# JackShDr/InfluentialRS

Measured on AMD Instinct MI355X. Metric: scored user-item pairs/sec (whole node), higher is better.
Workload: dtype f32; 1 GPU; c2: n_item=3415, d=128, L=200, H=4, layers=6, ffn=256; one greedy path-search step; users_per_gpu=4096, top_k=100, sweep=bf16 filter + exact f32 re-score, parallelism=single GPU

## Files before the change

influentialrs_amd/csrc/capi.hip:

```cpp
#include <stdlib.h>

#include <new>

#include "irs_internal.h"

int irs_launch_topk_exhaustive(irs_ctx *ctx, const float *xrows, int M, int k, float *val, int64_t *ids0,
                               int32_t *status, hipStream_t s);

static char g_create_err[512] = "";

static inline size_t align_up(size_t v, size_t a) { return (v + a - 1) / a * a; }

extern "C" int irs_abi_version(void) { return IRS_ABI_VERSION; }

extern "C" const char *irs_last_error(const irs_ctx *ctx) { return ctx ? ctx->err : g_create_err; }

extern "C" int irs_create(irs_ctx **out, const irs_dims *dims, const irs_shard *shard) {
    if (!out || !dims) {
        snprintf(g_create_err, sizeof(g_create_err), "irs_create: null argument");
        return IRS_E_INVALID;
    }
    const irs_dims &D = *dims;
#define BAD(...)                                                   \
    do {                                                           \
// ... 10 lines not shown
    if (D.mask_mode != IRS_MASK_IRN && D.mask_mode != IRS_MASK_CAUSAL) BAD("bad mask_mode");
    if (D.mask_mode == IRS_MASK_IRN && (D.u_dim < 1 || D.n_user < 1)) BAD("IRN mask needs user embeddings");
    if (D.max_rows < 1) BAD("max_rows must be >= 1");
    if (D.max_k < 1 || D.max_k > 1024) BAD("max_k must be in [1, 1024]");
    irs_shard sh;
    if (shard) sh = *shard;
    else {
        sh.rank = 0;
        sh.world = 1;
        sh.item_lo = 0;
        sh.item_hi = D.n_item;
    }
    if (sh.item_lo < 0 || sh.item_hi > D.n_item || sh.item_lo >= sh.item_hi) BAD("bad item shard [%lld, %lld)", (long long)sh.item_lo, (long long)sh.item_hi);
    if (sh.item_hi - sh.item_lo > 0x7FFFFFE0LL) BAD("shard too large");
    {
        int dev = 0;
        if (hipGetDevice(&dev) == hipSuccess && (dev < 0 || dev >= IRS_MAX_DEVICES))
            BAD("device ordinal %d: contexts are supported on devices 0 .. %d", dev, IRS_MAX_DEVICES - 1);
    }
#undef BAD
    irs_ctx *c = new (std::nothrow) irs_ctx();
    if (!c) {
        snprintf(g_create_err, sizeof(g_create_err), "out of host memory");
        return IRS_E_INVALID;
    }
    memset(c, 0, sizeof(*c));
    c->dims = D;
    c->shard = sh;
    c->n_local = sh.item_hi - sh.item_lo;
    int dp = 16;
    while (dp < D.d) dp <<= 1;
    c->d_pad = dp;
    c->KS = dp / 16;
    c->n_tiles = (int)((c->n_local + 31) / 32);
    c->max_rows = D.max_rows;
    c->max_seqs = D.max_seqs > 0 ? D.max_seqs : D.max_rows;
    c->m_pad_max = (c->max_rows + 31) & ~31;
    c->lse_slots = 2048;
    {
        const char *e = getenv("IRS_DECODER_GEMM");
        if (e && strcmp(e, "f32") && strcmp(e, "x6") && strcmp(e, "h3")) {
            snprintf(g_create_err, sizeof(g_create_err), "IRS_DECODER_GEMM=%s (expected h3, x6 or f32)", e);
            delete c;
            return IRS_E_INVALID;
        }
        c->use_x6 = e ? (strcmp(e, "f32") == 0 ? IRS_GEMM_F32 : strcmp(e, "x6") == 0 ? IRS_GEMM_X6 : IRS_GEMM_H3) : IRS_GEMM_H3;
        const char *ea = getenv("IRS_ATTN_GEMM");
        if (ea && strcmp(ea, "f32") && strcmp(ea, "h3")) {
            snprintf(g_create_err, sizeof(g_create_err), "IRS_ATTN_GEMM=%s (expected h3 or f32)", ea);
            delete c;
            return IRS_E_INVALID;
        }
        c->use_attn_h3 = ea ? (strcmp(ea, "h3") == 0) : 1;
        const char *es = getenv("IRS_DECODER_SEQ");
        c->use_seq = es ? (strcmp(es, "auto") == 0 ? 2 : (atoi(es) != 0 ? 1 : 0)) : 2;
        const char *ec = getenv("IRS_THR_CARRY");
        c->carry_period = ec ? atoi(ec) : 8;
        if (c->carry_period < 0 || c->carry_period > 1024) c->carry_period = 8;
        const char *eo = getenv("IRS_SHARDED_OVERLAP");
        c->sh_overlap = eo ? (atoi(eo) != 0 ? 1 : 0) : 0;
        const char *er = getenv("IRS_LSE_RING");
        c->lse_no_ring = er ? (strcmp(er, "0") == 0) : 0;
    }
    *out = c;
    return IRS_OK;
}

extern "C" void irs_destroy(irs_ctx *ctx) {
    if (!ctx) return;
    irs_drop_graphs(ctx);
    if (ctx->sh_side) {
        for (int i = 0; i < 8; ++i) (void)hipEventDestroy(ctx->sh_ev[i]);
        (void)hipStreamDestroy(ctx->sh_side);
    }
    if (ctx->prof_ev) {
        for (int i = 0; i < ctx->prof_cap; ++i) {
            hipEventDestroy(ctx->prof_ev[i].a);
            hipEventDestroy(ctx->prof_ev[i].b);
        }
        free(ctx->prof_ev);
    }
    delete ctx;
}

static bool ends_with(const char *s, const char *suf) {
    size_t ls = strlen(s), lf = strlen(suf);
    return ls >= lf && strcmp(s + ls - lf, suf) == 0;
}

extern "C" int irs_bind_weight(irs_ctx *ctx, const char *name, const float *p, int64_t numel) {
    if (!ctx || !name || !p) return IRS_E_INVALID;
    if (strncmp(name, "module.", 7) == 0) name += 7;
    const irs_dims &D = ctx->dims;
    const int64_t d = D.d, F = D.ffn_dim;
    const float **slot = nullptr;
    int64_t want = -1;
    if (!strcmp(name, "item_embedder.weight") || !strcmp(name, "word_embedder.weight")) {
        slot = &ctx->item_emb;
        want = (D.n_item + 1) * d;
    } else if (!strcmp(name, "user_embedder.weight")) {
        slot = &ctx->user_emb;
        want = D.n_user * D.u_dim;
    } else if (!strcmp(name, "pos_embedder.pe")) {
        slot = &ctx->pe;
        want = -2;
        if (numel < (int64_t)D.max_len * d) IRS_FAIL(ctx, IRS_E_INVALID, "pos_embedder.pe too small");
// ... 901 lines not shown
```

influentialrs_amd/csrc/irs_internal.h:

```cpp
#pragma once

#include <hip/hip_runtime.h>
#include <stdint.h>
#include <stdio.h>
#include <string.h>

#include "../../include/irs_hip.h"

#if !defined(IRS_LAB) && (defined(X6_DUMP) || defined(X6_STAMP) || defined(X6_NO_SPLIT) || defined(X6_STAGGER) ||            \
                          defined(X6_NO_MFMA) || defined(X6_NO_READS) || defined(X6_NO_DMA) || defined(X6_NO_BARRIER) ||       \
                          defined(X6_NW) || defined(ATTN_STAMP) || defined(ATTNP_STAMP) ||               \
                          defined(IRS_SMALL_TIMING) || defined(IRS_DIRECT_TIMING) || defined(SWEEP_LAB) || defined(X6D_STAMP) ||              \
                          defined(X6_NO_QKV_STORE) || defined(X6_NSLOT2) || defined(X6_RESID_LATE) || defined(X6_RING4) ||      \
                          defined(X6_SPLIT_ACC4) || defined(SEQ_EXP))
#error "a lab switch (X6_* / ATTN* / IRS_*_TIMING) is defined without IRS_LAB: the product library must be built without them"
#endif

#include <atomic>
#include <functional>
#define IRS_MAX_DEVICES 32
static inline int irs_cur_dev() {
    int d = 0;
    if (hipGetDevice(&d) != hipSuccess || d < 0 || d >= IRS_MAX_DEVICES) d = 0;
    return d;
// ... 12 lines not shown
#define IRS_CAND_BUCKETS 64
#define IRS_CAND_SLOTS 64
#define IRS_CAND_CAP (IRS_CAND_BUCKETS * IRS_CAND_SLOTS)
#define IRS_REFINE_CAP 1024
#define IRS_MAX_GROUPS 2048
#define IRS_MAX_PATH 64
#define IRS_LSE_SLOTS_RING 4096
#define IRS_COOP_FALLBACK_MIN_ITEMS 262144
#define IRS_EXH_SCRATCH_KEYS (64 * 32768)

struct irs_layer_w {
    const float *sa_in_w, *sa_in_b, *sa_out_w, *sa_out_b;
    const float *ca_in_w, *ca_in_b, *ca_out_w, *ca_out_b;
    const float *l1_w, *l1_b, *l2_w, *l2_b;
    const float *n1_w, *n1_b, *n2_w, *n2_b, *n3_w, *n3_b;
};

struct irs_prof_ev {
    hipEvent_t a, b;
};

enum { IRS_STEP_GREEDY = 1, IRS_STEP_BEAM, IRS_STEP_SHARDED_BEAM, IRS_STEP_SHARDED_BEAM_SPLIT };
struct irs_step_key {
    int32_t kind, B, W, P, k, sweep, sample, sample_k;
    uint64_t seed;
    const void *comm, *seq, *user, *hep, *paths, *status;
};
static_assert(sizeof(irs_step_key) == 8 * sizeof(int32_t) + 7 * 8, "irs_step_key is compared with memcmp: no padding");
struct irs_step_graph {
    hipGraphExec_t exec;
    irs_step_key key;
};

struct irs_ctx {
    irs_dims dims;
    irs_shard shard;
    int64_t n_local;
    int d_pad;
    int KS;
    int n_tiles;
    int max_seqs;
    int max_rows;
    int m_pad_max;

    const float *item_emb, *user_emb, *pe, *um_w, *um_b, *proj_w, *proj_b;
    irs_layer_w layer[IRS_MAX_LAYERS];

    uint4 *wp;
    float *bias_pad;
    float *c_l;
    float *wnorm_max;
    float *w_frag16;
    uint4 *w_x6;
    int use_x6;
    bool h3_ok;
    float h3_bound;
    int use_seq;
    bool seq_last;
    int32_t route_last[IRS_ROUTE_FIELDS];
    int route_n;
    int use_attn_h3;
    int lse_no_ring;
    bool finalized;
    bool proj_stale;

    char *ws;
    size_t ws_bytes;
    float *act_x, *act_y, *act_qkv, *act_ao, *act_h, *act_ru;
    float *act_qkv_b1;
    float *act_xf, *act_yf;
    int32_t *tok_row;
    int32_t *seq_cnt, *seq_off, *seq_qrow;
    int32_t *seq_padq;
    int32_t *m_dev;
    int32_t *tile_seq, *tile_idx;
    int32_t *seq_row0, *qrow_tile;
    int32_t *n_wg_dev;
    uint4 *xb;
    float *eps;
    float *thr;
    float *gm;
    unsigned int *cand_cnt;
    unsigned long long *cand;
    float *lse_part;
    int lse_slots;
    float *ref_tmp;
    int thr_valid, thr_M, thr_k, thr_age, carry_period;
    unsigned int *fb_count;
    int32_t *fb_list;
    unsigned long long *exh_keys;
    float *xrows;
    float *top_val;
    int64_t *top_ids;
    int32_t *row_status;
    int32_t *step_ctr;
    int32_t *step_pair;
    int32_t *pos_tmp;
    int64_t *bm_seq[2];
    int32_t *bm_hep[2];
    double *bm_cum[2];
    float *bm_paths[2];
    int64_t *bm_user;
    int64_t *bm_user2;
    int32_t *bm_fin[2];
    int32_t *bm_done[2];
    float *lse_max, *lse_sum;
// ... 318 lines not shown
```

influentialrs_amd/csrc/score.hip:

```cpp
#include <type_traits>

#include "irs_internal.h"

typedef __attribute__((ext_vector_type(16))) float f32x16;
typedef __attribute__((ext_vector_type(8))) __bf16 bf16x8;

#define MODE_PRE 0
#define MODE_EMIT 1
#define MODE_COUNT 2
#define MODE_DENSE 3
#define MODE_LSE 4
#define MODE_CEGRAD 5

struct SweepArgs {
    const uint4 *wp;
    const float *w32;
    const float *bias;
    const uint4 *xb;
    const float *x32;
    int M, M_pad, UT, d;
    int64_t n_local;
    int tile_begin, tile_end, tiles_per_wave, n_strips, n_ublocks;
    int tile_stride;
    int tiles_per_wg;
// ... 1350 lines not shown
}

__global__ void __launch_bounds__(256) k_pack_w(const float *__restrict__ W, const float *__restrict__ b, int64_t n_local,
                                                int n_tiles, int d, int KS, uint4 *__restrict__ wp,
                                                float *__restrict__ bias_pad, unsigned int *__restrict__ wn_bits) {
    int64_t row = (int64_t)blockIdx.x * 4 + (threadIdx.x >> 6);
    int lane = threadIdx.x & 63;
    if (row >= (int64_t)n_tiles * 32) return;
    const int64_t t = row >> 5;
    const int r = (int)(row & 31);
    float ss = 0.f, ssr = 0.f, ssd = 0.f;
    if (lane < 2 * KS) {
        uint4 v = pack8_bf16(W + (size_t)row * d, 8 * lane, d, row < n_local, ss, ssr, ssd);
        wp[((size_t)t * KS + (lane >> 1)) * 64 + (lane & 1) * 32 + r] = v;
    }
    ss = lanes_sum<63>(ss);
    ssr = lanes_sum<63>(ssr);
    ssd = lanes_sum<63>(ssd);
    if (lane == 0) {
        bias_pad[row] = (row < n_local) ? b[row] : -INFINITY;
        if (row < n_local) {
            atomicMax(wn_bits + 0, __float_as_uint(sqrtf(fmaxf(ss, ssr)) * 1.001f));
            atomicMax(wn_bits + 1, __float_as_uint(sqrtf(ssd) * 1.001f));
            atomicMax(wn_bits + 2, __float_as_uint(fabsf(b[row])));
        }
    }
}

#define SEL2_G IRS_MAX_GROUPS
static_assert(SEL2_G == 2048, "k_select_thr_bits: 32 keys per lane");
template <int CTRL>
__device__ __forceinline__ unsigned int dpp_u32(unsigned int v) {
    return (unsigned int)__builtin_amdgcn_update_dpp(0, (int)v, CTRL, 0xF, 0xF, true);
}
__device__ __forceinline__ unsigned int wave_sum_u32(unsigned int v) {
    v += dpp_u32<0xB1>(v);
    v += dpp_u32<0x4E>(v);
    v += dpp_u32<0x141>(v);
    v += dpp_u32<0x140>(v);
    return (unsigned int)__builtin_amdgcn_readlane((int)v, 0) + (unsigned int)__builtin_amdgcn_readlane((int)v, 16) +
           (unsigned int)__builtin_amdgcn_readlane((int)v, 32) + (unsigned int)__builtin_amdgcn_readlane((int)v, 48);
}
__device__ __forceinline__ unsigned int wave_max_u32(unsigned int v) {
    unsigned int o;
    o = dpp_u32<0xB1>(v), v = o > v ? o : v;
    o = dpp_u32<0x4E>(v), v = o > v ? o : v;
    o = dpp_u32<0x141>(v), v = o > v ? o : v;
    o = dpp_u32<0x140>(v), v = o > v ? o : v;
    const unsigned int a = (unsigned int)__builtin_amdgcn_readlane((int)v, 0), b = (unsigned int)__builtin_amdgcn_readlane((int)v, 16);
    const unsigned int c = (unsigned int)__builtin_amdgcn_readlane((int)v, 32), d = (unsigned int)__builtin_amdgcn_readlane((int)v, 48);
    const unsigned int ab = a > b ? a : b, cd = c > d ? c : d;
    return ab > cd ? ab : cd;
}
__global__ void __launch_bounds__(256) k_select_thr_bits(const float *__restrict__ gm, int G, int M, int M_pad, int k,
                                                         const float *__restrict__ eps, float *__restrict__ thr,
                                                         float *__restrict__ traw) {
    constexpr int STRIDE = SEL2_G + 16;
    constexpr int KPL = SEL2_G / 64;
    __shared__ unsigned int sel_lds[4 * STRIDE];
    const int tid = threadIdx.x;
    {
        const int rl = tid & 3, tq = tid >> 2;
        const int row = blockIdx.x * 4 + rl;
        const float *blk = gm + (size_t)blockIdx.x * G * 4 + rl;
        float raw[KPL];
#pragma unroll
        for (int i = 0; i < KPL; ++i) {
            const int g = tq + 64 * i;
            raw[i] = blk[(size_t)(g < G ? g : G - 1) * 4];
        }
#pragma unroll
        for (int i = 0; i < KPL; ++i) asm volatile("" : "+v"(raw[i]));
#pragma unroll
        for (int i = 0; i < KPL; ++i) {
            const int g = tq + 64 * i;
            const unsigned int kk = irs_fkey(raw[i]);
            sel_lds[rl * STRIDE + g] = (g < G && row < M) ? kk : 0u;
        }
    }
    __syncthreads();
    const int lane = tid & 63;
    const int wave = __builtin_amdgcn_readfirstlane(tid >> 6);
    const int row = blockIdx.x * 4 + wave;
    unsigned int key[KPL];
    unsigned int mx = 0u, mnc = 0u;
#pragma unroll
    for (int i = 0; i < KPL; ++i) {
        key[i] = sel_lds[wave * STRIDE + lane + 64 * i];
        mx = key[i] > mx ? key[i] : mx;
        const unsigned int c = (lane + 64 * i < G) ? ~key[i] : 0u;
        mnc = c > mnc ? c : mnc;
    }
    const unsigned int smx = wave_max_u32(mx), smn = ~wave_max_u32(mnc);
    const unsigned int diff = smx ^ smn;
    const int top = diff ? 31 - __builtin_clz(diff) : -1;
    unsigned int prefix = top >= 31 ? 0u : (smx & ~((2u << top) - 1u));
    if (top < 0) prefix = smx;
    for (int bit = top; bit >= 0; --bit) {
        const unsigned int cand = prefix | (1u << bit);
        unsigned int c0 = 0, c1 = 0, c2 = 0, c3 = 0;
#pragma unroll
        for (int i = 0; i < KPL; i += 4) {
            c0 += key[i] >= cand ? 1u : 0u;
            c1 += key[i + 1] >= cand ? 1u : 0u;
            c2 += key[i + 2] >= cand ? 1u : 0u;
            c3 += key[i + 3] >= cand ? 1u : 0u;
        }
        const unsigned int cnt = wave_sum_u32((c0 + c1) + (c2 + c3));
        if (cnt >= (unsigned int)k) prefix = cand;
    }
    if (lane == 0 && row < M_pad) {
// ... 130 lines not shown
            const unsigned long long key = keyfn(j);
            if (key > s_thr) {
                const unsigned int slot = atomicAdd(&s_n, 1u);
                buf[slot] = key;
            }
        }
        __syncthreads();
        if (s_n > EXH_BUF - 256) {
            const unsigned int n = s_n;
            for (int i = n + tid; i < EXH_BUF; i += 256) buf[i] = 0ull;
            bitonic_desc(buf, EXH_BUF);
            if (tid == 0) {
                s_n = (n < (unsigned int)k) ? n : k;
                if (n >= (unsigned int)k) s_thr = buf[k - 1];
            }
            __syncthreads();
        }
    }
    const unsigned int n = s_n;
    for (int i = n + tid; i < EXH_BUF; i += 256) buf[i] = 0ull;
    bitonic_desc(buf, EXH_BUF);
    __syncthreads();
    return n < (unsigned int)k ? n : (unsigned int)k;
}

__global__ void __launch_bounds__(256) k_exh_strips(const float *__restrict__ x, int d, const float *__restrict__ W,
                                                    const float *__restrict__ bias, int64_t n_local, int k, int n_strips,
                                                    const unsigned int *__restrict__ fb_count, const int32_t *__restrict__ fb_list,
                                                    unsigned long long *__restrict__ exh_keys) {
    __shared__ unsigned long long buf[EXH_BUF];
    __shared__ float xs[256];
    unsigned int nfb = *fb_count;
    if (nfb == 0u) return;
    if (nfb > EXH_FB_MAX) nfb = EXH_FB_MAX;
    const int strip = blockIdx.x;
    const int64_t per = (n_local + n_strips - 1) / n_strips;
    const int64_t j0 = (int64_t)strip * per, j1 = (j0 + per < n_local) ? j0 + per : n_local;
    for (unsigned int fi = blockIdx.y; fi < nfb; fi += gridDim.y) {
        const int row = fb_list[fi];
        __syncthreads();
        for (int i = threadIdx.x; i < d; i += 256) xs[i] = x[(size_t)row * d + i];
        __syncthreads();
        const unsigned int n = exh_select(
            [&](int64_t j) -> unsigned long long {
                const float e = irs_chain(xs, W + (size_t)j * d, bias[j], d);
                return ((unsigned long long)irs_fkey(e) << 32) | (0xFFFFFFFFu - (unsigned int)j);
            },
            j0, j1, k, buf);
        unsigned long long *o = exh_keys + ((size_t)fi * n_strips + strip) * k;
        for (int i = threadIdx.x; i < k; i += 256) o[i] = i < (int)n ? buf[i] : 0ull;
    }
}

__global__ void __launch_bounds__(256) k_refine(const float *__restrict__ x, int d, const float *__restrict__ W,
                                                const float *__restrict__ bias, const unsigned int *__restrict__ cnt,
                                                const unsigned long long *__restrict__ cand,
                                                const float *__restrict__ eps, const float *__restrict__ traw, int k,
                                                int64_t item_lo, int64_t n_local, float *__restrict__ val,
                                                int64_t *__restrict__ ids, int32_t *__restrict__ status,
                                                unsigned int *__restrict__ fb_count, int32_t *__restrict__ fb_list) {
    __shared__ __attribute__((aligned(16))) unsigned long long ckeys[IRS_CAND_CAP + 2];
    unsigned long long *rkeys = ckeys;
    __shared__ unsigned int hist[256];
    __shared__ float xs[256];
    __shared__ unsigned int boff[IRS_CAND_BUCKETS + 1];
    __shared__ unsigned int s_prefix, s_k, s_nr, s_above, s_over;
    const int row = blockIdx.x, tid = threadIdx.x;
    constexpr int PER = IRS_CAND_BUCKETS * IRS_CAND_SLOTS / 256;
    unsigned long long cv[PER];
#pragma unroll
    for (int j = 0; j < PER; ++j) {
        const int idx = tid + 256 * j;
        cv[j] = cand[((size_t)row * IRS_CAND_BUCKETS + idx / IRS_CAND_SLOTS) * IRS_CAND_SLOTS + idx % IRS_CAND_SLOTS];
    }
    for (int i = tid; i < d; i += 256) xs[i] = x[(size_t)row * d + i];
    if (tid < IRS_CAND_BUCKETS) hist[tid] = cnt[(size_t)row * IRS_CAND_BUCKETS + tid];
    __syncthreads();
    if (tid < 64) {
        const unsigned int cb = hist[tid] & ~IRS_CAND_OVERFLOW;
        const unsigned int cl = cb > IRS_CAND_SLOTS ? IRS_CAND_SLOTS : cb;
        unsigned int incl = cl;
#pragma unroll
        for (int o = 1; o < 64; o <<= 1) {
            const unsigned int t = __shfl_up(incl, o, 64);
            if (tid >= o) incl += t;
        }
        boff[tid] = incl - cl;
        if (tid == 63) boff[IRS_CAND_BUCKETS] = incl;
        const unsigned long long ov = __ballot((hist[tid] & IRS_CAND_OVERFLOW) != 0u);
        if (tid == 0) {
            s_over = ov ? 1u : 0u;
            s_prefix = 0;
            s_k = k;
            s_nr = 0;
            s_above = 0;
        }
    }
    __syncthreads();
    if (s_over) {
        if (tid == 0) status[row] |= IRS_ROW_FALLBACK;
        if (fb_count) {
            if (tid == 0) fb_list[atomicAdd(fb_count, 1u)] = row;
            return;
        }
        exhaustive_row(x, d, W, bias, n_local, item_lo, k, row, val, ids, status, ckeys, xs, true);
        return;
    }
    const unsigned int c = boff[IRS_CAND_BUCKETS];
#pragma unroll
    for (int j = 0; j < PER; ++j) {
        const int idx = tid + 256 * j;
        const int b = idx / IRS_CAND_SLOTS, sl = idx % IRS_CAND_SLOTS;
        if ((unsigned int)sl < boff[b + 1] - boff[b]) ckeys[boff[b] + sl] = cv[j];
    }
    __syncthreads();
    const float t1 = traw[row];
    if (t1 > -INFINITY) {
        unsigned int mine = 0;
        for (int i = tid; i < (int)c; i += 256) mine += (irs_unkey((unsigned int)(ckeys[i] >> 32)) >= t1) ? 1u : 0u;
        if (mine) atomicAdd(&s_above, mine);
// ... 31 lines not shown
            }
            __syncthreads();
            if (tid < 64) radix_find_bin(hist, s_k, tid, shift, &s_prefix, &s_k);
            __syncthreads();
        }
        thr2 = irs_unkey(s_prefix) - 2.0f * eps[row];
    }
    {
        constexpr int PERC = IRS_CAND_CAP / 256;
        unsigned int keep[PERC];
#pragma unroll
        for (int j = 0; j < PERC; ++j) {
            const int i = tid + 256 * j;
            keep[j] = 0xFFFFFFFFu;
            if (i < (int)c) {
                const unsigned long long key = ckeys[i];
                if (irs_unkey((unsigned int)(key >> 32)) >= thr2) keep[j] = (unsigned int)key;
            }
        }
        __syncthreads();
#pragma unroll
        for (int j = 0; j < PERC; ++j)
            if (keep[j] != 0xFFFFFFFFu) rkeys[atomicAdd(&s_nr, 1u)] = (unsigned long long)keep[j];
    }
    __syncthreads();
    const unsigned int nr = s_nr;
    for (int i = tid; i < (int)nr; i += 256) {
        unsigned int j = (unsigned int)rkeys[i];
        float e = irs_chain(xs, W + (size_t)j * d, bias[j], d);
        rkeys[i] = ((unsigned long long)irs_fkey(e) << 32) | (0xFFFFFFFFu - j);
    }
    if ((nr & 1) && tid == 0) rkeys[nr] = 0ull;
    __syncthreads();
    {
        const ulonglong2 *r2 = reinterpret_cast<const ulonglong2 *>(rkeys);
        for (int i = tid; i < (int)nr; i += 256) {
            const unsigned long long me = rkeys[i];
            int above = 0;
            for (int j = 0; j < (int)(nr + 1) / 2; ++j) {
                const ulonglong2 v = r2[j];
                above += (v.x > me) + (v.y > me);
            }
            if (above < k) {
                val[(size_t)row * k + above] = irs_unkey((unsigned int)(me >> 32));
                ids[(size_t)row * k + above] = item_lo + (int64_t)(0xFFFFFFFFu - (unsigned int)me);
            }
        }
        for (int i = (int)nr + tid; i < k; i += 256) {
            val[(size_t)row * k + i] = -INFINITY;
            ids[(size_t)row * k + i] = -1;
        }
    }
    if (tid == 0 && (int)nr < k) status[row] |= IRS_ROW_FEWER_THAN_K;
}

#define DIRECT_MAX_ITEMS 4096
#define DIRECT_TILE 64
#define DIRECT_MAX_D 256
#ifdef IRS_DIRECT_TIMING
__device__ unsigned long long g_direct_t[16];
#define DSTAMP(i) do { if (threadIdx.x == 0) tstamp[i] = __builtin_amdgcn_s_memtime(); } while (0)
#else
#define DSTAMP(i)
#endif
#define DIRECT_ROWS 8
template <int MODE>
__global__ void __launch_bounds__(256) k_topk_direct(const float *__restrict__ x, int d, const float *__restrict__ W,
                                                     const float *__restrict__ bias, int n_local, int64_t item_lo, int k,
                                                     unsigned long long *__restrict__ gkeys, unsigned int *__restrict__ arrive,
                                                     float *__restrict__ val, int64_t *__restrict__ ids,
                                                     int32_t *__restrict__ status, irs_path_args pa, int M) {
    __shared__ __attribute__((aligned(16))) float tile[DIRECT_TILE * (DIRECT_MAX_D + 4)];
    __shared__ __attribute__((aligned(16))) unsigned long long rkeys[IRS_REFINE_CAP + 2];
    __shared__ __attribute__((aligned(16))) float xs[(MODE == 1 ? DIRECT_ROWS : 1) * DIRECT_MAX_D];
    __shared__ __attribute__((aligned(16))) unsigned long long tmax[256];
    __shared__ unsigned int wsum[4];
    __shared__ unsigned int s_last, s_thr;
    const int row = MODE == 1 ? blockIdx.y * DIRECT_ROWS : blockIdx.y, tid = threadIdx.x, lane = tid & 63, wave = tid >> 6;
#ifdef IRS_DIRECT_TIMING
    unsigned long long tstamp[10];
#endif
    DSTAMP(0);
    unsigned int *gk = reinterpret_cast<unsigned int *>(gkeys + (size_t)row * IRS_CAND_CAP);
    if constexpr (MODE != 2) {
    const bool vec = (d & 3) == 0;
    const int S = vec ? ((d & 7) ? d : d + 4) : (d | 1);
    const int j0 = blockIdx.x * DIRECT_TILE;
    const int nj = min(DIRECT_TILE, n_local - j0);
    const int d4 = d >> 2;
    if (vec) {
        for (int i = tid; i < nj * d4; i += 256) {
            const int jj = i / d4, c4 = i - jj * d4;
            *reinterpret_cast<float4 *>(tile + jj * S + 4 * c4) = reinterpret_cast<const float4 *>(W + (size_t)j0 * d)[i];
        }
    } else {
        for (int i = tid; i < nj * d; i += 256) {
            const int jj = i / d, c = i - jj * d;
            tile[jj * S + c] = W[(size_t)j0 * d + i];
        }
    }
    if constexpr (MODE == 1) {
        for (int i = tid; i < DIRECT_ROWS * d; i += 256) {
            const int rr = i / d, c = i - rr * d;
            xs[rr * DIRECT_MAX_D + c] = (row + rr < M) ? x[(size_t)(row + rr) * d + c] : 0.f;
        }
        __syncthreads();
// ... 494 lines not shown
    }
    const bool xreg = a.UT == 1 && KS == 16;
    const int UB = xreg ? 1 : ub_f32(KS);
    a.n_ublocks = (a.UT + UB - 1) / UB;
    dim3 grid(((a.n_strips + 7) / 8) * 8 * a.n_ublocks);
    const size_t lds = (size_t)UB * KS * 2048 + EMIT_Q_BYTES;
#define L_(KS_, UB_, XR_)                                                                                                 \
    do {                                                                                                                  \
        IRS_ONCE_PER_DEVICE((void)hipFuncSetAttribute(reinterpret_cast<const void *>(k_lse_f32<KS_, UB_, EMIT, XR_>),     \
                                                      hipFuncAttributeMaxDynamicSharedMemorySize, (int)lds));             \
        hipLaunchKernelGGL((k_lse_f32<KS_, UB_, EMIT, XR_>), grid, dim3(256), lds, s, a);                                 \
    } while (0)
    switch (KS) {
    case 2: L_(2, 8, false); break;
    case 4: L_(4, 8, false); break;
    case 8: L_(8, 4, false); break;
    case 16: if (xreg) L_(16, 1, true); else L_(16, 2, false); break;
    default: IRS_FAIL(ctx, IRS_E_UNSUPPORTED, "unsupported d_pad %d", ctx->d_pad);
    }
#undef L_
    IRS_CHECK_HIP(ctx, hipGetLastError());
    return IRS_OK;
}

int irs_launch_pack_w(irs_ctx *ctx, hipStream_t s) {
    IRS_CHECK_HIP(ctx, hipMemsetAsync(ctx->wnorm_max, 0, 4 * sizeof(float), s));
    int64_t rows = (int64_t)ctx->n_tiles * 32;
    hipLaunchKernelGGL(k_pack_w, dim3((unsigned)((rows + 3) / 4)), dim3(256), 0, s, ctx->proj_w, ctx->proj_b,
                       ctx->n_local, ctx->n_tiles, ctx->dims.d, ctx->KS, ctx->wp,
                       ctx->bias_pad, reinterpret_cast<unsigned int *>(ctx->wnorm_max));
    IRS_CHECK_HIP(ctx, hipGetLastError());
    return IRS_OK;
}

bool irs_topk_is_direct(const irs_ctx *ctx, int M, int k) {
    return M <= 1024 && ctx->n_local <= DIRECT_MAX_ITEMS && k <= 256 && ctx->dims.d <= DIRECT_MAX_D;
}

enum TopkForm {
    TOPK_DIRECT1,
    TOPK_DIRECT2,
    TOPK_SWEPT,
};
struct TopkPlan {
    TopkForm form;
    bool fused_lse;
    bool lse_after;
    bool reuse_thr;
    bool coop_fb;
    int stride;
    int nt0;
    int tpw0;
    int r_sel;
};

static TopkPlan topk_plan(const irs_ctx *ctx, const float *xrows, int M, int k, int sweep, bool want_lse, int carry) {
    TopkPlan p{};
    if (irs_topk_is_direct(ctx, M, k)) {
        p.form = M <= 32 ? TOPK_DIRECT1 : TOPK_DIRECT2;
        p.lse_after = want_lse;
        return p;
    }
    p.form = TOPK_SWEPT;
    SweepArgs a;
    sweep_common(ctx, a, xrows, M);
    p.fused_lse = want_lse && sweep == IRS_SWEEP_BF16 && lse_fast_ok(ctx, a);
    p.lse_after = want_lse && !p.fused_lse;
    p.coop_fb = ctx->n_local >= IRS_COOP_FALLBACK_MIN_ITEMS && ctx->exh_keys != nullptr;
    const int nt = ctx->n_tiles;
    p.reuse_thr = carry && ctx->carry_period > 0 && sweep == IRS_SWEEP_BF16 && !p.fused_lse && ctx->thr_valid && ctx->thr_M == M &&
                  ctx->thr_k == k && ctx->thr_age + 1 < ctx->carry_period && nt >= 2 * 8 * 1024;
    if (p.reuse_thr) return p;
    int nt0 = nt >= 16 * 1024 ? nt / 16 : nt / 8;
    if (nt0 < 1024) nt0 = 1024;
    if (nt0 > nt) nt0 = nt;
    p.stride = nt / nt0;
    p.nt0 = (nt + p.stride - 1) / p.stride;
    p.tpw0 = (p.nt0 + 1023) / 1024;
    p.r_sel = k;
    if (p.stride > 1) {
        p.r_sel = ((p.stride >= 16 ? 4 : 3) * k + p.stride - 1) / p.stride;
        if (p.r_sel < 8) p.r_sel = 8;
        if (p.r_sel > k) p.r_sel = k;
    }
    return p;
}

static int topk_direct(irs_ctx *ctx, const TopkPlan &p, const float *xrows, int M, int k, float *val, int64_t *ids0,
                       int32_t *status, const irs_path_args *path, hipStream_t s) {
    irs_prof_begin(ctx, IRS_PROF_REFINE, s);
    const unsigned int tiles = (unsigned)((ctx->n_local + DIRECT_TILE - 1) / DIRECT_TILE);
    unsigned int *arrive = reinterpret_cast<unsigned int *>(ctx->step_ctr) + 8;
    const irs_path_args pa = path ? *path : irs_path_args{};
    if (p.form == TOPK_DIRECT1)
        hipLaunchKernelGGL(k_topk_direct<0>, dim3(tiles, M), dim3(256), 0, s, xrows, ctx->dims.d, ctx->proj_w, ctx->proj_b,
                           (int)ctx->n_local, ctx->shard.item_lo, k, ctx->cand, arrive, val, ids0, status, pa, M);
    else {
        hipLaunchKernelGGL(k_topk_direct<1>, dim3(tiles, (M + DIRECT_ROWS - 1) / DIRECT_ROWS), dim3(256), 0, s, xrows, ctx->dims.d,
                           ctx->proj_w, ctx->proj_b, (int)ctx->n_local, ctx->shard.item_lo, k, ctx->cand, arrive, val, ids0,
                           status, irs_path_args{}, M);
        hipLaunchKernelGGL(k_topk_direct<2>, dim3(1, M), dim3(256), 0, s, xrows, ctx->dims.d, ctx->proj_w, ctx->proj_b,
                           (int)ctx->n_local, ctx->shard.item_lo, k, ctx->cand, arrive, val, ids0, status, pa, M);
    }
    irs_prof_end(ctx, IRS_PROF_REFINE, s, 2.0 * ctx->dims.d * (double)M * (double)ctx->n_local, 0.0);
    IRS_CHECK_HIP(ctx, hipGetLastError());
    return IRS_OK;
}

static int topk_prep(irs_ctx *ctx, const TopkPlan &p, const float *xrows, int M, int M_pad, int sweep, int32_t *status,
                     hipStream_t s) {
    static_assert(IRS_CAND_BUCKETS == 64, "k_prep_x resets one bucket counter per lane");
    if (sweep == IRS_SWEEP_BF16) {
        const float acc_factor = (float)(ctx->d_pad + 8) * 2.384185791015625e-07f;
        hipLaunchKernelGGL(k_prep_x, dim3((M_pad + 3) / 4), dim3(256), 0, s, xrows, M, M_pad, ctx->dims.d, ctx->KS,
                           ctx->xb, ctx->eps, ctx->wnorm_max, acc_factor, ctx->cand_cnt, status, p.coop_fb ? ctx->fb_count : nullptr,
                           p.reuse_thr ? ctx->thr : nullptr, p.reuse_thr ? ctx->ref_tmp : nullptr);
    } else {
        IRS_CHECK_HIP(ctx, hipMemsetAsync(status, 0, sizeof(int32_t) * M, s));
        IRS_CHECK_HIP(ctx, hipMemsetAsync(ctx->cand_cnt, 0, sizeof(unsigned int) * (size_t)M_pad * IRS_CAND_BUCKETS, s));
        hipLaunchKernelGGL(k_zero_eps, dim3((M_pad + 255) / 256), dim3(256), 0, s, ctx->eps, M_pad);
    }
    IRS_CHECK_HIP(ctx, hipGetLastError());
    return IRS_OK;
}

static int topk_select(irs_ctx *ctx, const TopkPlan &p, SweepArgs &a, int M, int sweep, hipStream_t s) {
    sweep_decompose(a, 0, ctx->n_tiles, 1, p.tpw0, p.stride);
    const int G = 2 * a.n_strips * 4;
    if (G > SEL2_G) IRS_FAIL(ctx, IRS_E_UNSUPPORTED, "pre-pass groups %d > %d", G, SEL2_G);
    a.gm = ctx->gm;
    a.n_groups = G;
    irs_prof_begin(ctx, IRS_PROF_SWEEP, s);
    const int rc = sweep == IRS_SWEEP_BF16 ? launch_sweep_bf16<MODE_PRE>(ctx, a, s) : launch_sweep_f32<MODE_PRE>(ctx, a, s);
    irs_prof_end(ctx, IRS_PROF_SWEEP, s, 2.0 * ctx->dims.d * (double)M * p.nt0 * 32.0,
                 (double)p.nt0 * 32.0 * ctx->d_pad * (sweep == IRS_SWEEP_BF16 ? 2.0 : 4.0));
    if (rc) return rc;
    hipLaunchKernelGGL(k_select_thr_bits, dim3((a.M_pad + 3) / 4), dim3(256), 0, s, ctx->gm, G, M, a.M_pad, p.r_sel, ctx->eps,
                       ctx->thr, ctx->ref_tmp);
    IRS_CHECK_HIP(ctx, hipGetLastError());
    return IRS_OK;
}

static int topk_emit(irs_ctx *ctx, const TopkPlan &p, SweepArgs &a, int M, int sweep, float *lse_max, float *lse_sum,
                     hipStream_t s) {
    a.thr = ctx->thr;
    a.cnt = ctx->cand_cnt;
    a.cand = ctx->cand;
    int lse_slots = 0, rc;
    if (p.fused_lse) {
        if ((rc = lse_decompose(ctx, a, &lse_slots))) return rc;
    } else {
        const int UB = sweep == IRS_SWEEP_BF16 ? ub_bf16(ctx->KS) : ub_f32(ctx->KS);
        sweep_decompose(a, 0, ctx->n_tiles, (a.UT + UB - 1) / UB, 0);
    }
    const double flops = 2.0 * ctx->dims.d * (double)M * (double)ctx->n_local;
    const double bytes = (double)ctx->n_tiles * 32.0 * ctx->d_pad * ((sweep == IRS_SWEEP_BF16 && !p.fused_lse) ? 2.0 : 4.0);
    irs_prof_begin(ctx, IRS_PROF_SWEEP, s);
    irs_prof_begin(ctx, IRS_PROF_SWEEP_EMIT, s);
    if (p.fused_lse) rc = launch_lse_f32<true>(ctx, a, s);
    else if (sweep == IRS_SWEEP_BF16) rc = launch_sweep_bf16<MODE_EMIT>(ctx, a, s);
    else rc = launch_sweep_f32<MODE_EMIT>(ctx, a, s);
    irs_prof_end(ctx, IRS_PROF_SWEEP, s, flops, bytes);
    irs_prof_end(ctx, IRS_PROF_SWEEP_EMIT, s, flops, bytes);
    if (rc) return rc;
    if (p.fused_lse) {
        hipLaunchKernelGGL(k_lse_reduce, dim3(M), dim3(256), 0, s, ctx->lse_part, lse_slots, a.M_pad, M, lse_max, lse_sum);
        IRS_CHECK_HIP(ctx, hipGetLastError());
    }
    return IRS_OK;
}

static int topk_refine(irs_ctx *ctx, const TopkPlan &p, const float *xrows, int M, int k, int sweep, float *val, int64_t *ids0,
                       int32_t *status, hipStream_t s) {
    const int d = ctx->dims.d;
    irs_prof_begin(ctx, IRS_PROF_REFINE, s);
    if (p.coop_fb && sweep != IRS_SWEEP_BF16) IRS_CHECK_HIP(ctx, hipMemsetAsync(ctx->fb_count, 0, sizeof(unsigned int), s));
    hipLaunchKernelGGL(k_refine, dim3(M), dim3(256), 0, s, xrows, d, ctx->proj_w, ctx->proj_b, ctx->cand_cnt, ctx->cand,
                       ctx->eps, ctx->ref_tmp, k, ctx->shard.item_lo, ctx->n_local, val, ids0, status,
                       p.coop_fb ? ctx->fb_count : nullptr, ctx->fb_list);
    if (p.coop_fb) {
        int ns = EXH_STRIPS;
        while (ns > 1 && (long long)ns * k > EXH_KEYS_PER_ROW) ns >>= 1;
        hipLaunchKernelGGL(k_exh_strips, dim3(ns, 4), dim3(256), 0, s, xrows, d, ctx->proj_w, ctx->proj_b, ctx->n_local, k, ns,
                           ctx->fb_count, ctx->fb_list, ctx->exh_keys);
        hipLaunchKernelGGL(k_exh_merge, dim3(EXH_FB_MAX), dim3(256), 0, s, xrows, d, ctx->proj_w, ctx->proj_b, ctx->n_local,
                           ctx->shard.item_lo, k, ns, ctx->fb_count, ctx->fb_list, ctx->exh_keys, val, ids0, status);
    }
    irs_prof_end(ctx, IRS_PROF_REFINE, s, 0.0, 0.0);
    IRS_CHECK_HIP(ctx, hipGetLastError());
    return IRS_OK;
}

int irs_launch_topk(irs_ctx *ctx, const float *xrows, int M, int k, int sweep, float *val, int64_t *ids0,
                    int32_t *status, hipStream_t s, const irs_path_args *path, float *lse_max, float *lse_sum, int carry) {
    const TopkPlan p = topk_plan(ctx, xrows, M, k, sweep, lse_max != nullptr, carry);
    if (path && p.form == TOPK_SWEPT) IRS_FAIL(ctx, IRS_E_STATE, "fused path step needs the direct top-k");
    int rc;
    if (p.form != TOPK_SWEPT) {
        if ((rc = topk_direct(ctx, p, xrows, M, k, val, ids0, status, path, s))) return rc;
    } else {
        SweepArgs a;
        sweep_common(ctx, a, xrows, M);
        if ((rc = topk_prep(ctx, p, xrows, M, a.M_pad, sweep, status, s))) return rc;
        if (p.reuse_thr) ++ctx->thr_age;
        else {
            if ((rc = topk_select(ctx, p, a, M, sweep, s))) return rc;
            ctx->thr_valid = sweep == IRS_SWEEP_BF16, ctx->thr_M = M, ctx->thr_k = k, ctx->thr_age = 0;
        }
        if ((rc = topk_emit(ctx, p, a, M, sweep, lse_max, lse_sum, s))) return rc;
        if ((rc = topk_refine(ctx, p, xrows, M, k, sweep, val, ids0, status, s))) return rc;
    }
    return p.lse_after ? irs_launch_lse(ctx, xrows, M, lse_max, lse_sum, s) : IRS_OK;
}

int irs_launch_topk_exhaustive(irs_ctx *ctx, const float *xrows, int M, int k, float *val, int64_t *ids0,
                               int32_t *status, hipStream_t s) {
    IRS_CHECK_HIP(ctx, hipMemsetAsync(status, 0, sizeof(int32_t) * M, s));
    hipLaunchKernelGGL(k_exhaustive, dim3(M), dim3(256), 0, s, xrows, ctx->dims.d, ctx->proj_w, ctx->proj_b,
                       ctx->n_local, ctx->shard.item_lo, k, 0, val, ids0, status);
    IRS_CHECK_HIP(ctx, hipGetLastError());
    return IRS_OK;
}

int irs_launch_gather(irs_ctx *ctx, const float *xrows, int M, const int64_t *ids0, int g, float *out, hipStream_t s) {
    hipLaunchKernelGGL(k_gather, dim3(M), dim3(64), 0, s, xrows, ctx->dims.d, ctx->proj_w, ctx->proj_b,
                       ctx->shard.item_lo, ctx->n_local, ids0, g, out);
    IRS_CHECK_HIP(ctx, hipGetLastError());
    return IRS_OK;
}

int irs_launch_count_before(irs_ctx *ctx, const float *xrows, int M, const float *ref_score, const int64_t *ref_id0,
                            const int64_t *excl, int n_excl, int64_t *count, hipStream_t s) {
// ... 137 lines not shown
```

Measured before the change: 2.208 billion pairs/s.

## Add wave-per-row top-k refine and narrow threshold select for small group counts

Adds k_refine_wave, which handles four rows per block with one wavefront each. Each wave gathers the candidates, finds the threshold by radix bit search using wave reductions, re-scores the survivors in f32, and ranks them by counting. Rows that overflow or hit the capacity limit fall back to the existing block-per-row refine. A templated k_select_thr_bits with a smaller keys-per-lane count is used when the group count fits. Both paths are on by default for the bf16 stride-1 non-LSE sweep and can be turned off with IRS_TOPK_ONE_SWEEP=0. The aim is to cut per-row block overhead and __syncthreads in refine; the cost is a smaller per-wave candidate capacity and an O(nr²) rank step.

```diff
diff --git a/influentialrs_amd/csrc/capi.hip b/influentialrs_amd/csrc/capi.hip
--- a/influentialrs_amd/csrc/capi.hip
+++ b/influentialrs_amd/csrc/capi.hip
@@ -86,6 +86,13 @@
             return IRS_E_INVALID;
         }
         c->use_attn_h3 = ea ? (strcmp(ea, "h3") == 0) : 1;
+        const char *et = getenv("IRS_TOPK_ONE_SWEEP");
+        if (et && strcmp(et, "0") && strcmp(et, "1")) {
+            snprintf(g_create_err, sizeof(g_create_err), "IRS_TOPK_ONE_SWEEP=%s (expected 0 or 1)", et);
+            delete c;
+            return IRS_E_INVALID;
+        }
+        c->topk_tight = et ? (strcmp(et, "1") == 0) : 1;
         const char *es = getenv("IRS_DECODER_SEQ");
         c->use_seq = es ? (strcmp(es, "auto") == 0 ? 2 : (atoi(es) != 0 ? 1 : 0)) : 2;
         const char *ec = getenv("IRS_THR_CARRY");
diff --git a/influentialrs_amd/csrc/irs_internal.h b/influentialrs_amd/csrc/irs_internal.h
--- a/influentialrs_amd/csrc/irs_internal.h
+++ b/influentialrs_amd/csrc/irs_internal.h
@@ -88,6 +88,7 @@
     float *wnorm_max;
     float *w_frag16;
     uint4 *w_x6;
+    int topk_tight;
     int use_x6;
     bool h3_ok;
     float h3_bound;
diff --git a/influentialrs_amd/csrc/score.hip b/influentialrs_amd/csrc/score.hip
--- a/influentialrs_amd/csrc/score.hip
+++ b/influentialrs_amd/csrc/score.hip
@@ -1426,11 +1426,12 @@
     const unsigned int ab = a > b ? a : b, cd = c > d ? c : d;
     return ab > cd ? ab : cd;
 }
+template <int KPL>
 __global__ void __launch_bounds__(256) k_select_thr_bits(const float *__restrict__ gm, int G, int M, int M_pad, int k,
                                                          const float *__restrict__ eps, float *__restrict__ thr,
                                                          float *__restrict__ traw) {
-    constexpr int STRIDE = SEL2_G + 16;
-    constexpr int KPL = SEL2_G / 64;
+    static_assert(KPL % 4 == 0 && KPL * 64 <= SEL2_G, "four partial counts; at most IRS_MAX_GROUPS keys");
+    constexpr int STRIDE = KPL * 64 + 16;
     __shared__ unsigned int sel_lds[4 * STRIDE];
     const int tid = threadIdx.x;
     {
@@ -1667,20 +1668,18 @@
     }
 }
 
-__global__ void __launch_bounds__(256) k_refine(const float *__restrict__ x, int d, const float *__restrict__ W,
-                                                const float *__restrict__ bias, const unsigned int *__restrict__ cnt,
-                                                const unsigned long long *__restrict__ cand,
-                                                const float *__restrict__ eps, const float *__restrict__ traw, int k,
-                                                int64_t item_lo, int64_t n_local, float *__restrict__ val,
-                                                int64_t *__restrict__ ids, int32_t *__restrict__ status,
-                                                unsigned int *__restrict__ fb_count, int32_t *__restrict__ fb_list) {
-    __shared__ __attribute__((aligned(16))) unsigned long long ckeys[IRS_CAND_CAP + 2];
+__device__ __forceinline__ void refine_row(const float *__restrict__ x, int d, const float *__restrict__ W,
+                                           const float *__restrict__ bias, const unsigned int *__restrict__ cnt,
+                                           const unsigned long long *__restrict__ cand, const float *__restrict__ eps,
+                                           const float *__restrict__ traw, int k, int64_t item_lo, int64_t n_local,
+                                           float *__restrict__ val, int64_t *__restrict__ ids, int32_t *__restrict__ status,
+                                           unsigned int *__restrict__ fb_count, int32_t *__restrict__ fb_list, const int row,
+                                           unsigned long long *ckeys, float *xs) {
     unsigned long long *rkeys = ckeys;
     __shared__ unsigned int hist[256];
-    __shared__ float xs[256];
     __shared__ unsigned int boff[IRS_CAND_BUCKETS + 1];
     __shared__ unsigned int s_prefix, s_k, s_nr, s_above, s_over;
-    const int row = blockIdx.x, tid = threadIdx.x;
+    const int tid = threadIdx.x;
     constexpr int PER = IRS_CAND_BUCKETS * IRS_CAND_SLOTS / 256;
     unsigned long long cv[PER];
 #pragma unroll
@@ -1818,6 +1817,149 @@
         }
     }
     if (tid == 0 && (int)nr < k) status[row] |= IRS_ROW_FEWER_THAN_K;
+}
+
+__global__ void __launch_bounds__(256) k_refine(const float *__restrict__ x, int d, const float *__restrict__ W,
+                                                const float *__restrict__ bias, const unsigned int *__restrict__ cnt,
+                                                const unsigned long long *__restrict__ cand,
+                                                const float *__restrict__ eps, const float *__restrict__ traw, int k,
+                                                int64_t item_lo, int64_t n_local, float *__restrict__ val,
+                                                int64_t *__restrict__ ids, int32_t *__restrict__ status,
+                                                unsigned int *__restrict__ fb_count, int32_t *__restrict__ fb_list) {
+    __shared__ __attribute__((aligned(16))) unsigned long long ckeys[IRS_CAND_CAP + 2];
+    __shared__ float xs[256];
+    refine_row(x, d, W, bias, cnt, cand, eps, traw, k, item_lo, n_local, val, ids, status, fb_count, fb_list, (int)blockIdx.x,
+               ckeys, xs);
+}
+
+#define RW_CAP (IRS_CAND_CAP / 4)
+#define RW_PER (RW_CAP / 64)
+__device__ __forceinline__ void wave_lds_sync() {
+    __builtin_amdgcn_fence(__ATOMIC_ACQ_REL, "wavefront");
+    __builtin_amdgcn_wave_barrier();
+}
+__global__ void __launch_bounds__(256) k_refine_wave(const float *__restrict__ x, int d, const float *__restrict__ W,
+                                                     const float *__restrict__ bias, const unsigned int *__restrict__ cnt,
+                                                     const unsigned long long *__restrict__ cand,
+                                                     const float *__restrict__ eps, const float *__restrict__ traw, int k,
+                                                     int64_t item_lo, int64_t n_local, float *__restrict__ val,
+                                                     int64_t *__restrict__ ids, int32_t *__restrict__ status,
+                                                     unsigned int *__restrict__ fb_count, int32_t *__restrict__ fb_list, int M) {
+    __shared__ __attribute__((aligned(16))) unsigned long long ckeys[IRS_CAND_CAP + 2];
+    __shared__ float xs4[4 * 256];
+    __shared__ unsigned int woff[4][IRS_CAND_BUCKETS + 1];
+    __shared__ unsigned int s_slow[4];
+    const int tid = threadIdx.x, lane = tid & 63;
+    const int wave = __builtin_amdgcn_readfirstlane(tid >> 6);
+    const int row = blockIdx.x * 4 + wave;
+    unsigned long long *wk = ckeys + wave * RW_CAP;
+    float *xs = xs4 + wave * 256;
+    bool slow = false;
+    if (row < M) {
+        const unsigned int h = cnt[(size_t)row * IRS_CAND_BUCKETS + lane];
+        for (int i = lane; i < d; i += 64) xs[i] = x[(size_t)row * d + i];
+        const float t1 = traw[row], e2 = eps[row];
+        const unsigned int cb = h & ~IRS_CAND_OVERFLOW;
+        const unsigned int cl = cb > IRS_CAND_SLOTS ? IRS_CAND_SLOTS : cb;
+        unsigned int incl = cl;
+#pragma unroll
+        for (int o = 1; o < 64; o <<= 1) {
+            const unsigned int t = __shfl_up(incl, o, 64);
+            if (lane >= o) incl += t;
+        }
+        woff[wave][lane] = incl - cl;
+        if (lane == 63) woff[wave][IRS_CAND_BUCKETS] = incl;
+        const unsigned int c = (unsigned int)__builtin_amdgcn_readlane((int)incl, 63);
+        slow = __ballot((h & IRS_CAND_OVERFLOW) != 0u) != 0ull || c >= RW_CAP;
+        if (!slow) {
+            wave_lds_sync();
+            unsigned int khi[RW_PER], klo[RW_PER];
+#pragma unroll
+            for (int j = 0; j < RW_PER; ++j) {
+                const unsigned int i = (unsigned int)lane + 64u * j;
+                khi[j] = 0u;
+                klo[j] = 0u;
+                if (64u * j < c && i < c) {
+                    unsigned int b = 0u;
+#pragma unroll
+                    for (unsigned int st = IRS_CAND_BUCKETS / 2; st; st >>= 1)
+                        if (woff[wave][b + st] <= i) b += st;
+                    const unsigned long long key = cand[((size_t)row * IRS_CAND_BUCKETS + b) * IRS_CAND_SLOTS + (i - woff[wave][b])];
+                    khi[j] = (unsigned int)(key >> 32);
+                    klo[j] = (unsigned int)key;
+                }
+            }
+            if (t1 > -INFINITY) {
+                unsigned int mine = 0u;
+#pragma unroll
+                for (int j = 0; j < RW_PER; ++j)
+                    if (64u * j < c) mine += ((unsigned int)lane + 64u * j < c && irs_unkey(khi[j]) >= t1) ? 1u : 0u;
+                if (wave_sum_u32(mine) < (unsigned int)k) slow = true;
+            }
+            if (!slow) {
+                float thr2 = -INFINITY;
+                if (c >= (unsigned int)k) {
+                    unsigned int prefix = 0u;
+                    for (int bit = 31; bit >= 0; --bit) {
+                        const unsigned int cd = prefix | (1u << bit);
+                        unsigned int mine = 0u;
+#pragma unroll
+                        for (int j = 0; j < RW_PER; ++j)
+                            if (64u * j < c) mine += khi[j] >= cd ? 1u : 0u;
+                        if (wave_sum_u32(mine) >= (unsigned int)k) prefix = cd;
+                    }
+                    thr2 = irs_unkey(prefix) - 2.0f * e2;
+                }
+                unsigned int nr = 0u;
+#pragma unroll
+                for (int j = 0; j < RW_PER; ++j) {
+                    if (64u * j < c) {
+                        const bool keep = (unsigned int)lane + 64u * j < c && irs_unkey(khi[j]) >= thr2;
+                        const unsigned long long m = __ballot(keep);
+                        if (keep)
+                            wk[__builtin_amdgcn_mbcnt_hi((unsigned int)(m >> 32), __builtin_amdgcn_mbcnt_lo((unsigned int)m, nr))] =
+                                (unsigned long long)klo[j];
+                        nr += (unsigned int)__popcll(m);
+                    }
+                }
+                wave_lds_sync();
+                for (int i = lane; i < (int)nr; i += 64) {
+                    const unsigned int j = (unsigned int)wk[i];
+                    const float e = irs_chain(xs, W + (size_t)j * d, bias[j], d);
+                    wk[i] = ((unsigned long long)irs_fkey(e) << 32) | (0xFFFFFFFFu - j);
+                }
+                if ((nr & 1u) && lane == 0) wk[nr] = 0ull;
+                wave_lds_sync();
+                const ulonglong2 *r2 = reinterpret_cast<const ulonglong2 *>(wk);
+                for (int i = lane; i < (int)nr; i += 64) {
+                    const unsigned long long me = wk[i];
+                    int above = 0;
+                    for (int j = 0; j < (int)(nr + 1) / 2; ++j) {
+                        const ulonglong2 v = r2[j];
+                        above += (v.x > me) + (v.y > me);
+                    }
+                    if (above < k) {
+                        val[(size_t)row * k + above] = irs_unkey((unsigned int)(me >> 32));
+                        ids[(size_t)row * k + above] = item_lo + (int64_t)(0xFFFFFFFFu - (unsigned int)me);
+                    }
+                }
+                for (int i = (int)nr + lane; i < k; i += 64) {
+                    val[(size_t)row * k + i] = -INFINITY;
+                    ids[(size_t)row * k + i] = -1;
+                }
+                if (lane == 0 && (int)nr < k) status[row] |= IRS_ROW_FEWER_THAN_K;
+            }
+        }
+    }
+    if (lane == 0) s_slow[wave] = slow ? 1u : 0u;
+    __syncthreads();
+    for (int w = 0; w < 4; ++w) {
+        if (s_slow[w]) {
+            refine_row(x, d, W, bias, cnt, cand, eps, traw, k, item_lo, n_local, val, ids, status, fb_count, fb_list,
+                       (int)blockIdx.x * 4 + w, ckeys, xs4);
+            __syncthreads();
+        }
+    }
 }
 
 #define DIRECT_MAX_ITEMS 4096
@@ -2418,6 +2560,7 @@
     int nt0;
     int tpw0;
     int r_sel;
+    bool tight;
 };
 
 static TopkPlan topk_plan(const irs_ctx *ctx, const float *xrows, int M, int k, int sweep, bool want_lse, int carry) {
@@ -2449,6 +2592,7 @@
         if (p.r_sel < 8) p.r_sel = 8;
         if (p.r_sel > k) p.r_sel = k;
     }
+    p.tight = ctx->topk_tight && p.stride == 1 && sweep == IRS_SWEEP_BF16 && !p.fused_lse;
     return p;
 }
 
@@ -2501,8 +2645,12 @@
     irs_prof_end(ctx, IRS_PROF_SWEEP, s, 2.0 * ctx->dims.d * (double)M * p.nt0 * 32.0,
                  (double)p.nt0 * 32.0 * ctx->d_pad * (sweep == IRS_SWEEP_BF16 ? 2.0 : 4.0));
     if (rc) return rc;
-    hipLaunchKernelGGL(k_select_thr_bits, dim3((a.M_pad + 3) / 4), dim3(256), 0, s, ctx->gm, G, M, a.M_pad, p.r_sel, ctx->eps,
-                       ctx->thr, ctx->ref_tmp);
+    if (p.tight && G <= 4 * 64)
+        hipLaunchKernelGGL(k_select_thr_bits<4>, dim3((a.M_pad + 3) / 4), dim3(256), 0, s, ctx->gm, G, M, a.M_pad, p.r_sel,
+                           ctx->eps, ctx->thr, ctx->ref_tmp);
+    else
+        hipLaunchKernelGGL(k_select_thr_bits<SEL2_G / 64>, dim3((a.M_pad + 3) / 4), dim3(256), 0, s, ctx->gm, G, M, a.M_pad,
+                           p.r_sel, ctx->eps, ctx->thr, ctx->ref_tmp);
     IRS_CHECK_HIP(ctx, hipGetLastError());
     return IRS_OK;
 }
@@ -2541,9 +2689,14 @@
     const int d = ctx->dims.d;
     irs_prof_begin(ctx, IRS_PROF_REFINE, s);
     if (p.coop_fb && sweep != IRS_SWEEP_BF16) IRS_CHECK_HIP(ctx, hipMemsetAsync(ctx->fb_count, 0, sizeof(unsigned int), s));
-    hipLaunchKernelGGL(k_refine, dim3(M), dim3(256), 0, s, xrows, d, ctx->proj_w, ctx->proj_b, ctx->cand_cnt, ctx->cand,
-                       ctx->eps, ctx->ref_tmp, k, ctx->shard.item_lo, ctx->n_local, val, ids0, status,
-                       p.coop_fb ? ctx->fb_count : nullptr, ctx->fb_list);
+    if (p.tight)
+        hipLaunchKernelGGL(k_refine_wave, dim3((M + 3) / 4), dim3(256), 0, s, xrows, d, ctx->proj_w, ctx->proj_b, ctx->cand_cnt,
+                           ctx->cand, ctx->eps, ctx->ref_tmp, k, ctx->shard.item_lo, ctx->n_local, val, ids0, status,
+                           p.coop_fb ? ctx->fb_count : nullptr, ctx->fb_list, M);
+    else
+        hipLaunchKernelGGL(k_refine, dim3(M), dim3(256), 0, s, xrows, d, ctx->proj_w, ctx->proj_b, ctx->cand_cnt, ctx->cand,
+                           ctx->eps, ctx->ref_tmp, k, ctx->shard.item_lo, ctx->n_local, val, ids0, status,
+                           p.coop_fb ? ctx->fb_count : nullptr, ctx->fb_list);
     if (p.coop_fb) {
         int ns = EXH_STRIPS;
         while (ns > 1 && (long long)ns * k > EXH_KEYS_PER_ROW) ns >>= 1;
```

After: 2.218 billion pairs/s, median of 6. About the same (+0.5%).
